# jeffsonyu/VTacO

Hardware: AMD Instinct MI355X
Metric: occupancy query-points/sec at 128^3 (decode stage, lattice -> logits on device) (higher is better)
Workload: dtype f16x3

## Files before the change

### include/vtaco_hip.h

```cpp
#ifndef VTACO_HIP_H
#define VTACO_HIP_H

#include <stddef.h>
#include <stdint.h>

#ifdef __cplusplus
extern "C" {
#endif

#define VT_ABI_VERSION 1

#define VT_ERR_INVALID      (-1)
#define VT_ERR_UNSUPPORTED  (-2)
#define VT_ERR_WORKSPACE    (-3)

#define VT_MAX_BLOCKS 8

int         vt_abi_version(void);
const char *vt_last_error(void);

typedef struct vt_decoder_params {
    int32_t hidden;
    int32_t c_dim;
    int32_t n_blocks;
// ... 38 lines not shown
                        int lattice_nx, float lattice_box, int64_t lattice_first,
                        const float *c_img, const unsigned char *finger_ids, const float *finger_feats, int F,
                        const float *blob_f16x3, double padding, float *out, float *out2, void *stream);

int vt_decoder_pack_f16f8(const vt_decoder_params *params_host, float *blob, size_t blob_bytes, void *stream);
int vt_decode_f16f8_covers(int R, int C, int lattice_nx, float lattice_box, int64_t lattice_first, int64_t N, double padding);
int vt_decode_fwd_f16f8(const float *grid_cl, int B, int R, int C, int64_t N,
                        int lattice_nx, float lattice_box, int64_t lattice_first,
                        const float *c_img, const unsigned char *finger_ids, const float *finger_feats, int F,
                        const float *blob_f16f8, double padding, float *out, void *stream);

int vt_decode_range_status(unsigned *host_status, int reset, void *stream);

int vt_decode_last_clock(unsigned long long *shader_cycles, unsigned long long *ref_ticks, int *ref_khz,
                         unsigned long long *wg_ticks, int max_wgs, int *n_wgs, void *stream);

#define VT_WIDE_LEAKY 1
#define VT_WIDE_NEAREST 2
size_t vt_decoder_wide_blob_bytes(int hidden, int c_dim, int n_blocks, int p_in);
int vt_decoder_pack_wide(const vt_decoder_params *params_host, float *blob, size_t blob_bytes, void *stream);
int vt_decode_fwd_wide(const float *grid_cl, int B, int R, int C, const float *pts, int64_t N,
                       int lattice_nx, float lattice_box, int64_t lattice_first,
                       const float *c_img, const float *blob_wide, int hidden, int n_blocks, int flags, double padding,
                       float *out, float *out2, void *stream);
size_t vt_decoder_wide_blob_f16x3_bytes(int hidden, int c_dim, int n_blocks, int p_in);
int vt_decoder_pack_wide_f16x3(const vt_decoder_params *params_host, float *blob, size_t blob_bytes, void *stream);
int vt_decode_fwd_wide_f16x3(const float *grid_cl, int B, int R, int C, const float *pts, int64_t N,
                             int lattice_nx, float lattice_box, int64_t lattice_first,
                             const float *c_img, const float *blob_wide_f16x3, int hidden, int n_blocks, int flags, double padding,
                             float *out, float *out2, void *stream);
// ... 488 lines not shown
```

### vtaco_amd/_lib.py

```python
from __future__ import annotations

import ctypes
import os

import torch

_HERE = os.path.dirname(os.path.abspath(__file__))
LIB_PATH = os.environ.get("VTACO_HIP_LIB") or os.path.join(_HERE, "libvtaco_hip.so")

VT_MAX_BLOCKS = 8
c_float_p = ctypes.POINTER(ctypes.c_float)


class VtError(RuntimeError):
    pass


class DecoderParams(ctypes.Structure):
    _fields_ = [
        ("hidden", ctypes.c_int32), ("c_dim", ctypes.c_int32),
        ("n_blocks", ctypes.c_int32), ("p_in", ctypes.c_int32),
        ("fc_p_w", ctypes.c_void_p), ("fc_p_b", ctypes.c_void_p),
        ("fc_c_w", ctypes.c_void_p * VT_MAX_BLOCKS), ("fc_c_b", ctypes.c_void_p * VT_MAX_BLOCKS),
        ("fc0_w", ctypes.c_void_p * VT_MAX_BLOCKS), ("fc0_b", ctypes.c_void_p * VT_MAX_BLOCKS),
# ... 117 lines not shown
    "vt_fusion_fwd_train": (_I, [_VP, _VP, _I, _I, ctypes.POINTER(FusionParams), _F, ctypes.c_ulonglong, _VP, _SZ, _VP, _SZ, _VP, _VP]),
    "vt_fusion_bwd": (_I, [_VP, _VP, _VP, _I, _I, ctypes.POINTER(FusionParams), _F, ctypes.c_ulonglong, _VP, _SZ, _VP, _SZ, _VP, _VP,
                           ctypes.POINTER(FusionGrads), _VP]),
    "vt_fusion_dropout_mask": (_I, [_F, ctypes.c_ulonglong, _I, _I, _I, _VP, _VP]),
    "vt_fusion_saved_bytes_wide": (_SZ, [_I, _I, _I]),
    "vt_fusion_bwd_workspace_bytes_wide": (_SZ, [_I, _I, _I]),
    "vt_fusion_dropout_mask_wide": (_I, [_F, ctypes.c_ulonglong, _I, _I, _I, _I, _VP, _VP]),
    "vt_decoder_blob_t_bytes": (_SZ, [_I, _I, _I]),
    "vt_decoder_pack_bf16x3": (_I, [ctypes.POINTER(DecoderParams), _VP, _SZ, _VP]),
    "vt_decode_fwd_bf16x3": (_I, [_VP, _I, _I, _I, _VP, _I64, _I, _F, _I64, _VP, _VP, _VP, _I, _VP, _D, _VP, _VP, _VP]),
    "vt_decoder_pack_f16x3": (_I, [ctypes.POINTER(DecoderParams), _VP, _SZ, _VP]),
    "vt_decode_fwd_f16x3": (_I, [_VP, _I, _I, _I, _VP, _I64, _I, _F, _I64, _VP, _VP, _VP, _I, _VP, _D, _VP, _VP, _VP]),
    "vt_decode_range_status": (_I, [ctypes.POINTER(ctypes.c_uint32), _I, _VP]),
    "vt_decode_last_clock": (_I, [ctypes.POINTER(ctypes.c_uint64), ctypes.POINTER(ctypes.c_uint64), ctypes.POINTER(ctypes.c_int),
                                  ctypes.POINTER(ctypes.c_uint64), _I, ctypes.POINTER(ctypes.c_int), _VP]),
    "vt_decoder_pack_f16f8": (_I, [ctypes.POINTER(DecoderParams), _VP, _SZ, _VP]),
    "vt_decoder_wide_blob_bytes": (_SZ, [_I, _I, _I, _I]),
    "vt_decoder_wide_blob_f16x3_bytes": (_SZ, [_I, _I, _I, _I]),
    "vt_decoder_pack_wide": (_I, [ctypes.POINTER(DecoderParams), _VP, _SZ, _VP]),
    "vt_decoder_pack_wide_f16x3": (_I, [ctypes.POINTER(DecoderParams), _VP, _SZ, _VP]),
    "vt_decode_fwd_wide": (_I, [_VP, _I, _I, _I, _VP, _I64, _I, _F, _I64, _VP, _VP, _I, _I, _I, _D, _VP, _VP, _VP]),
    "vt_decode_fwd_wide_f16x3": (_I, [_VP, _I, _I, _I, _VP, _I64, _I, _F, _I64, _VP, _VP, _I, _I, _I, _D, _VP, _VP, _VP]),
    "vt_decode_fwd_wide_ids": (_I, [_VP, _I, _I, _I, _VP, _I64, _I, _F, _I64, _VP, _VP, _I, _VP, _I, _I, _I, _D, _VP, _VP, _VP]),
    "vt_decode_wide_f16x3_workspace_bytes": (_SZ, [_I64, _I, _I, _I, _I]),
    "vt_decode_fwd_wide_f16x3_ws": (_I, [_VP, _I, _I, _I, _VP, _I64, _I, _F, _I64, _VP, _VP, _I, _I, _I, _D, _VP, _VP, _VP, _SZ, _VP]),
    "vt_decode_fwd_wide_f16x3_ids": (_I, [_VP, _I, _I, _I, _VP, _I64, _I, _F, _I64, _VP, _VP, _I, _VP, _I, _I, _I, _D, _VP, _VP, _VP]),
    "vt_decode_mlp_fwd_wide": (_I, [_VP, _I, _I, _VP, _I64, _I, _F, _I64, _VP, _I, _I, _I, _VP, _VP, _VP]),
    "vt_decode_mlp_fwd_wide_f16x3": (_I, [_VP, _I, _I, _VP, _I64, _I, _F, _I64, _VP, _I, _I, _I, _VP, _VP, _VP]),
    "vt_decode_wide_save_floats": (_SZ, [_I64, _I, _I, _I]),
    "vt_decode_wide_gws_floats": (_SZ, [_I64, _I, _I, _I]),
# ... 207 lines not shown
```

### vtaco_amd/csrc/decode.hip

```cpp
#include <hip/hip_runtime.h>
#include <atomic>
#include <mutex>
#include <type_traits>
#include <stdint.h>
#include <stdlib.h>

#include "decode_common.h"

namespace {

template <bool SAVE, int P>
__device__ __forceinline__ void mlp_and_heads(const DecodeArgs &a, const float *L, const f32x16 &c, float px, float py, float pz,
                                              uint32_t g, bool live, int lane, int h, bool with_img, unsigned &rmax) {
    const size_t slot = (size_t)a.total * 32;
    float *srow = SAVE ? a.save + (size_t)g * 32 : nullptr;
    if (SAVE && live) store_gather16(srow, c, h);

    f32x16 net = load_frag16(L + VT_OFF_BIAS + 0 * 32 + h * 16);
    {
        const float k0 = h ? py : px;
        const float k1 = h ? 0.0f : pz;
        net = mfma(L[VT_OFF_WP + lane], k0, net);
        net = mfma(L[VT_OFF_WP + 64 + lane], k1, net);
    }
// ... 368 lines not shown
    const int R = a.R;
    AxisEnt *tab = reinterpret_cast<AxisEnt *>(lds + VT_BLOB_FLOATS);
    for (int i = threadIdx.x; i < a.nx; i += ST2_THREADS) {
        float p, unused0, unused1;
        lattice_point(a, (uint32_t)i, 0u, 0u, p, unused0, unused1);
        const float f = grid_coord(p, a.divisor, R);
        const float f0 = floorf(f);
        AxisEnt e;
        e.i0 = (int)f0;
        e.w0 = (f0 + 1.0f) - f;
        e.i1 = min(e.i0 + 1, R - 1);
        e.w1 = (e.i0 + 1 <= R - 1) ? f - f0 : 0.0f;
        tab[i] = e;
    }
    unsigned *claim_ctr = reinterpret_cast<unsigned *>(reinterpret_cast<char *>(lds + VT_BLOB_FLOATS + 4 * a.nx) + (ST2_THREADS / 64) * ST2_WAVE_BYTES);
    if (threadIdx.x == 0) *claim_ctr = 0u;
    __syncthreads();

    const int lane = threadIdx.x & 63;
    const int pl = lane & 31;
    const int h = lane >> 5;
    const int wave = __builtin_amdgcn_readfirstlane(threadIdx.x >> 6);
    constexpr int WPB = ST2_THREADS / 64;
    const uint32_t ntiles = a.total >> 6;
    const uint32_t nx = (uint32_t)a.nx;
    const uint32_t tpb = a.N >> 6, q4 = nx >> 2, q8 = nx >> 3;
    const uint32_t plane0 = a.lattice_first / (nx * nx);
    char *stage = reinterpret_cast<char *>(lds + VT_BLOB_FLOATS + 4 * a.nx) + wave * ST2_WAVE_BYTES;

    uint32_t src_off[ST2_PIECES], dst_off[ST2_PIECES];
#pragma unroll
// ... 208 lines not shown
                netB = netB + bb;
            }
        }
        {
            const f32x16 wo = load_frag16(L + VT_OFF_OUT + h * 16);
            float accA = 0.0f, accB = 0.0f;
#pragma unroll
            for (int s = 0; s < 16; ++s) { accA = fmaf(relu1(netA[s]), wo[s], accA); accB = fmaf(relu1(netB[s]), wo[s], accB); }
            accA += __shfl_xor(accA, 32);
            accB += __shfl_xor(accB, 32);
            const float ob = L[VT_OFF_OUT + 64];
            if (h == 0) { a.out[gA] = accA + ob; a.out[gB] = accB + ob; }
        }
    }
    if constexpr (P == 2) range_report(rmax, a.status);
    clock_end(a.clk, stamp, reinterpret_cast<unsigned long long *>(claim_ctr + 4));
}

}
#ifdef VT_DECODE_F16_TU
#include "decode_st3.h"
#endif
namespace {

#ifndef VT_DECODE_F16_TU
__global__ void __launch_bounds__(256) sample_grid_kernel(DecodeArgs a, float *feat, int C) {
    const int lane = threadIdx.x & 63, pl = lane & 31, h = lane >> 5;
    const uint32_t ntiles = (a.total + 31u) >> 5;
    const int R = a.R;
    for (uint32_t tile = blockIdx.x * 4 + (threadIdx.x >> 6); tile < ntiles; tile += gridDim.x * 4) {
        uint32_t g = tile * 32u + pl;
// ... 196 lines not shown
        if (c0 + c < C && v0 + v < V) t[v][c] = s[(v0 + v) * C + c0 + c];
    }
    __syncthreads();
    for (int i = threadIdx.x; i < 32 * 64; i += 256) {
        const int c = i >> 6, v = i & 63;
        if (c0 + c < C && v0 + v < V) d[(int64_t)c * V + v0 + v] = t[v][c];
    }
}

#endif

}

#ifndef VT_DECODE_F16_TU
constexpr int VT_MAX_DEVICES = 64;
constexpr size_t VT_STATUS_BYTES = 8 + (4 + 2 * VT_CLK_MAX_WGS) * 8;
static std::mutex g_status_mutex;
static std::atomic<unsigned *> g_decode_status[VT_MAX_DEVICES];
unsigned *vt_decode_status_dev() {
    int dev = -1;
    if (hipGetDevice(&dev) != hipSuccess || dev < 0 || dev >= VT_MAX_DEVICES) return nullptr;
    unsigned *p = g_decode_status[dev].load(std::memory_order_acquire);
    if (p) return p;
    std::lock_guard<std::mutex> lock(g_status_mutex);
    p = g_decode_status[dev].load(std::memory_order_relaxed);
    if (!p) {
        if (hipMalloc(&p, VT_STATUS_BYTES) != hipSuccess) return nullptr;
        if (hipMemset(p, 0, VT_STATUS_BYTES) != hipSuccess) { (void)hipFree(p); return nullptr; }
        g_decode_status[dev].store(p, std::memory_order_release);
    }
    return p;
// ... 82 lines not shown
    if (e == hipSuccess) e = hipStreamSynchronize((hipStream_t)stream);
    int dev = 0, khz = 0;
    if (e == hipSuccess) e = hipGetDevice(&dev);
    if (e == hipSuccess) e = hipDeviceGetAttribute(&khz, hipDeviceAttributeWallClockRate, dev);
    if (e != hipSuccess) return vt_check(e, "vt_decode_last_clock");
    *shader_cycles = h[0]; *ref_ticks = h[1]; *ref_khz = khz;
    if (max_wgs > 0) {
        int n = (int)(h[2] < (unsigned long long)VT_CLK_MAX_WGS ? h[2] : VT_CLK_MAX_WGS);
        if (n > max_wgs) n = max_wgs;
        for (int i = 0; i < 2 * n; ++i) wg_ticks[i] = h[4 + i];
        *n_wgs = n;
    }
    return 0;
}

int vt_grid_to_channels_last(const float *src, float *dst, int B, int C, int D, int H, int W, void *stream) {
    if (!src || !dst || B <= 0 || C <= 0 || D <= 0 || H <= 0 || W <= 0) return vt_fail(VT_ERR_INVALID, "vt_grid_to_channels_last: bad argument");
    const int64_t V = (int64_t)D * H * W;
    dim3 grid((unsigned)((V + 63) / 64), (unsigned)((C + 31) / 32), (unsigned)B);
    hipLaunchKernelGGL(grid_to_cl_kernel, grid, dim3(256), 0, (hipStream_t)stream, src, dst, C, V);
    return vt_check(hipGetLastError(), "vt_grid_to_channels_last");
}

int vt_grid_from_channels_last(const float *src, float *dst, int B, int C, int D, int H, int W, void *stream) {
    if (!src || !dst || B <= 0 || C <= 0 || D <= 0 || H <= 0 || W <= 0) return vt_fail(VT_ERR_INVALID, "vt_grid_from_channels_last: bad argument");
    const int64_t V = (int64_t)D * H * W;
    dim3 grid((unsigned)((V + 63) / 64), (unsigned)((C + 31) / 32), (unsigned)B);
    hipLaunchKernelGGL(grid_from_cl_kernel, grid, dim3(256), 0, (hipStream_t)stream, src, dst, C, V);
    return vt_check(hipGetLastError(), "vt_grid_from_channels_last");
}
// ... 2 lines not shown
#endif

#ifdef VT_DECODE_F16_TU
static bool st3_covers(int nx, int R, double s_vox) {
    const size_t lds = ((size_t)VT_BLOB_FLOATS + 5u * (size_t)nx) * sizeof(float) + (size_t)(ST3_THREADS / 64) * ST2_WAVE_BYTES + VT_TAIL_LDS_BYTES;
    return (nx & 7) == 0 && R >= 6 && s_vox > 0.0 && s_vox < 0.55 && lds <= 160u * 1024u;
}
static int st3_launch(const DecodeArgs &a_in, int variant, void *stream) {
    DecodeArgs a = a_in;
    a.clk = status_clk(a.status);
    const size_t lds = ((size_t)VT_BLOB_FLOATS + 5u * (size_t)a.nx) * sizeof(float) + (size_t)(ST3_THREADS / 64) * ST2_WAVE_BYTES + VT_TAIL_LDS_BYTES;
    const int64_t nt = (int64_t)a.total / 64;
    int64_t blocks = (nt + ST3_THREADS / 64 - 1) / (ST3_THREADS / 64);
    if (blocks > vt_num_cus()) blocks = vt_num_cus();
    if (blocks > 8) blocks &= ~7ll;
    bool attr = false;
    if (!attr) {
        hipError_t e = vt_max_dyn_lds(reinterpret_cast<const void *>(&decode_fwd_staged3_kernel<0>), 160 * 1024);
        if (e == hipSuccess) e = vt_max_dyn_lds(reinterpret_cast<const void *>(&decode_fwd_staged3_kernel<1>), 160 * 1024);
        if (e == hipSuccess) e = vt_max_dyn_lds(reinterpret_cast<const void *>(&decode_fwd_staged3_kernel<2>), 160 * 1024);
        if (e == hipSuccess) e = vt_max_dyn_lds(reinterpret_cast<const void *>(&decode_fwd_staged3_kernel<3>), 160 * 1024);
        if (e != hipSuccess) return vt_check(e, "vt_decode_fwd: hipFuncSetAttribute (staged3)");
        attr = true;
    }
    if (variant == 0) hipLaunchKernelGGL(decode_fwd_staged3_kernel<0>, dim3((unsigned)blocks), dim3(ST3_THREADS), lds, (hipStream_t)stream, a);
    else if (variant == 1) hipLaunchKernelGGL(decode_fwd_staged3_kernel<1>, dim3((unsigned)blocks), dim3(ST3_THREADS), lds, (hipStream_t)stream, a);
    else if (variant == 2) hipLaunchKernelGGL(decode_fwd_staged3_kernel<2>, dim3((unsigned)blocks), dim3(ST3_THREADS), lds, (hipStream_t)stream, a);
    else hipLaunchKernelGGL(decode_fwd_staged3_kernel<3>, dim3((unsigned)blocks), dim3(ST3_THREADS), lds, (hipStream_t)stream, a);
    return vt_check(hipGetLastError(), "vt_decode_fwd");
}
static double lattice_step_voxels(int R, int nx, float box, double padding) {
    return (double)(R - 1) * (double)box / ((double)(nx - 1) * (double)(float)(1.0 + padding + 10e-4));
}
int vt_st3_sample_lattice(const float *grid_cl, int B, int R, int C, int64_t N, int nx, float box, int64_t first, double padding,
                          float *feat, void *stream, int *covered) {
    *covered = 0;
    if (C != 32 || nx < 8 || N <= 0 || (int64_t)B * N >= (int64_t)1 << 31) return 0;
    const int64_t pair = 2ll * nx * nx;
// ... 243 lines not shown
```

### vtaco_amd/csrc/decode_common.h

```cpp
#pragma once
#include <hip/hip_runtime.h>
#include <stdint.h>

#include "vt_common.h"

namespace {

typedef float f32x16 __attribute__((ext_vector_type(16)));
typedef float f32x4 __attribute__((ext_vector_type(4)));

__device__ __forceinline__ f32x16 mfma(float a, float b, f32x16 c) {
    return __builtin_amdgcn_mfma_f32_32x32x2f32(a, b, c, 0, 0, 0);
}

__device__ __forceinline__ float relu1(float x) {
    return __builtin_amdgcn_fmed3f(x, 0.0f, __builtin_inff());
}

__device__ __forceinline__ void pin16(f32x16 &v) {
    asm volatile("" : "+v"(v));
}

template <bool RELU>
__device__ __forceinline__ f32x16 dense32(f32x16 acc, const float *wl, const f32x16 &x, int lane) {
// ... 99 lines not shown
}

constexpr int VT_CLK_MAX_WGS = 512;
constexpr unsigned VT_TAIL_LDS_BYTES = 256;
struct ClockStamp {
    unsigned long long t0, r0;
};
__device__ __forceinline__ ClockStamp clock_begin(const unsigned long long *clk) {
    ClockStamp c{0ull, 0ull};
    if (clk != nullptr) {
        c.r0 = __builtin_amdgcn_s_memrealtime();
        if (blockIdx.x == 0) c.t0 = __builtin_readcyclecounter();
    }
    return c;
}
__device__ __forceinline__ void clock_end(unsigned long long *clk, const ClockStamp &c, unsigned long long *wave_ends) {
    if (clk != nullptr) {
        const unsigned long long r1 = __builtin_amdgcn_s_memrealtime();
        const unsigned long long dt = blockIdx.x == 0 ? __builtin_readcyclecounter() - c.t0 : 0ull;
        const int nwaves = (int)(blockDim.x >> 6);
        if ((threadIdx.x & 63) == 0) wave_ends[threadIdx.x >> 6] = r1;
        __syncthreads();
        if (threadIdx.x == 0) {
            unsigned long long last = r1;
            for (int w = 1; w < nwaves; ++w) last = wave_ends[w] > last ? wave_ends[w] : last;
            if (blockIdx.x == 0) { clk[0] = dt; clk[1] = r1 - c.r0; clk[2] = gridDim.x; }
            if (blockIdx.x < VT_CLK_MAX_WGS) { clk[4 + 2 * blockIdx.x] = c.r0; clk[5 + 2 * blockIdx.x] = last; }
        }
    }
}

template <int P>
__device__ __forceinline__ f32x16 dense32s(f32x16 acc, const float *wl, const SplitP<P> &x, int lane) {
    const mx8<P> *w = reinterpret_cast<const mx8<P> *>(wl);
#pragma unroll
    for (int s = 0; s < 2; ++s) {
        const mx8<P> wh = w[s * 64 + lane], wo = w[(2 + s) * 64 + lane];
        acc = mfma_s(wo, x.hi[s], acc);
        acc = mfma_s(wh, x.lo[s], acc);
        acc = mfma_s(wh, x.hi[s], acc);
    }
    return acc;
// ... 136 lines not shown
```

### vtaco_amd/csrc/decode_st3.h

```cpp
#pragma once

namespace {

typedef unsigned u32x8 __attribute__((ext_vector_type(8)));
typedef int i32x8 __attribute__((ext_vector_type(8)));
typedef short i16x2 __attribute__((ext_vector_type(2)));

constexpr int ST3_F8_SX = VT_F8_SX;
constexpr int ST3_F8_SW = VT_F8_SW;

template <int V> struct SpT {
    u32x4 hi[2], lo[2];
};
template <> struct SpT<2> {
    u32x4 hi[2];
    u32x8 q;
};

__device__ __forceinline__ f32x16 mfma_h(const u32x4 &a, const u32x4 &b, f32x16 c) {
    return __builtin_amdgcn_mfma_f32_32x32x16_f16(__builtin_bit_cast(f16x8, a), __builtin_bit_cast(f16x8, b), c, 0, 0, 0);
}
__device__ __forceinline__ f32x16 mfma_q(const u32x8 &a, const u32x8 &b, f32x16 c) {
    return __builtin_amdgcn_mfma_scale_f32_32x32x64_f8f6f4(__builtin_bit_cast(i32x8, a), __builtin_bit_cast(i32x8, b), c, 0, 0,
                                                           0, 127 - 11 - ST3_F8_SW, 0, 127 + ST3_F8_SX);
// ... 96 lines not shown
static_assert(ST3_CHUNKS - 64 * ST3_PIECES == 8, "the last LDS-DMA piece is eight lanes");

#define ST3_GAP() __builtin_amdgcn_sched_barrier(0)
#define ST3_M(acc, w, x) do { acc = mfma_h(w, x, acc); ST3_GAP(); } while (0)
#define ST3_Q(acc, w, x) do { acc = mfma_q(w, x, acc); ST3_GAP(); } while (0)
#define ST3_RUN_BLOCKS() do { _Pragma("unroll 1") for (int i = 0; i < 4; ++i) block(i, std::true_type{}); block(4, std::false_type{}); } while (0)
#define ST3_S(dst, src, k) split_step<V, true, k>(dst, src, m1, rmax)
#define ST3_C(dst, src, k) split_step<V, false, k>(dst, src, m1, rmax)

template <int V>
__global__ void __launch_bounds__(ST3_THREADS)
decode_fwd_staged3_kernel(DecodeArgs a) {
    extern __shared__ __attribute__((aligned(16))) float lds[];
    const ClockStamp stamp = clock_begin(a.clk);
    if constexpr (V == 2) __builtin_amdgcn_s_setreg((1 - 1) << 11 | 23 << 6 | 1, 1);
    if constexpr (V != 3) {
        const f32x4 *src = reinterpret_cast<const f32x4 *>(a.blob);
        f32x4 *dst = reinterpret_cast<f32x4 *>(lds);
        for (int i = threadIdx.x; i < VT_BLOB_FLOATS / 4; i += ST3_THREADS) dst[i] = src[i];
    }
    const int R = a.R;
    AxisEnt *tab = reinterpret_cast<AxisEnt *>(lds + VT_BLOB_FLOATS);
    unsigned *ptab = reinterpret_cast<unsigned *>(tab + a.nx);
    for (int i = threadIdx.x; i < a.nx; i += ST3_THREADS) {
        float p, unused0, unused1;
        lattice_point(a, (uint32_t)i, 0u, 0u, p, unused0, unused1);
        const float f = grid_coord(p, a.divisor, R);
        const float f0 = floorf(f);
        AxisEnt e;
        e.i0 = (int)f0;
        e.w0 = (f0 + 1.0f) - f;
        e.i1 = min(e.i0 + 1, R - 1);
        e.w1 = (e.i0 + 1 <= R - 1) ? f - f0 : 0.0f;
        tab[i] = e;
        const _Float16 ph = (_Float16)p;
        const _Float16 pm = (_Float16)(p - (float)ph);
        ptab[i] = (unsigned)__builtin_bit_cast(unsigned short, ph) | ((unsigned)__builtin_bit_cast(unsigned short, pm) << 16);
    }
    if (threadIdx.x == 0)
        *reinterpret_cast<unsigned *>(reinterpret_cast<char *>(lds + VT_BLOB_FLOATS + 5 * a.nx) + (ST3_THREADS / 64) * ST2_WAVE_BYTES) = 0u;
    __syncthreads();

    const int lane = threadIdx.x & 63;
    const int pl = lane & 31;
    const int h = lane >> 5;
    const int wave = __builtin_amdgcn_readfirstlane(threadIdx.x >> 6);
    constexpr int WPB = ST3_THREADS / 64;
    const uint32_t ntiles = a.total >> 6;
    const uint32_t nx = (uint32_t)a.nx;
    const uint32_t tpb = a.N >> 6, q4 = nx >> 2, q8 = nx >> 3;
    const uint32_t plane0 = a.lattice_first / (nx * nx);
    char *stage = reinterpret_cast<char *>(lds + VT_BLOB_FLOATS + 5 * a.nx) + wave * ST2_WAVE_BYTES;
    unsigned *claim_ctr = reinterpret_cast<unsigned *>(reinterpret_cast<char *>(lds + VT_BLOB_FLOATS + 5 * a.nx) + WPB * ST2_WAVE_BYTES);
    const unsigned stage_lds = (unsigned)__builtin_amdgcn_readfirstlane((int)(unsigned)reinterpret_cast<size_t>(stage));
    const unsigned stage_lds_last = (unsigned)__builtin_amdgcn_readfirstlane((int)(stage_lds + 1024u * ST3_PIECES));

    uint32_t src_off[ST3_PIECES + 1];
#pragma unroll
    for (int k = 0; k <= ST3_PIECES; ++k) {
        const int m = min(64 * k + lane, ST3_CHUNKS - 1), row = m / 9, c = m - 9 * row;
        const int dx = row % 3, t = row / 3, dy = t & 3, dz = t >> 2;
        src_off[k] = (uint32_t)((dz * R + dy) * R + dx) * 128u + (uint32_t)((c == 8) ? 0 : c) * 16u;
    }

    uint32_t t_begin = 0, t_end = ntiles, w_idx = blockIdx.x * WPB + wave, w_cnt = gridDim.x * WPB;
    if ((gridDim.x & 7u) == 0 && ntiles >= 8u * WPB) {
        const uint32_t chunk = (ntiles + 7u) >> 3, xcd = blockIdx.x & 7u;
        t_begin = min(xcd * chunk, ntiles);
        t_end = min(t_begin + chunk, ntiles);
        w_idx = (blockIdx.x >> 3) * WPB + wave;
        w_cnt = (gridDim.x >> 3) * WPB;
    }
    auto brick_of = [&](uint32_t tile, uint32_t &b, uint32_t &X0, uint32_t &Y0, uint32_t &Z0) {
        b = tile / tpb;
        const uint32_t t = tile - b * tpb;
        const uint32_t pp = t / (q4 * q8), rem = t - pp * q4 * q8;
        const uint32_t by = rem / q8, bz = rem - by * q8;
        X0 = 2u * pp; Y0 = 4u * by; Z0 = 8u * bz;
    };
    int ox = 0, oy = 0, oz = 0;
    auto fetch = [&](uint32_t tile, int &fx, int &fy, int &fz) {
        uint32_t b, X0, Y0, Z0;
        brick_of(tile, b, X0, Y0, Z0);
        fx = min(__builtin_amdgcn_readfirstlane(tab[plane0 + X0].i0), R - 3);
        fy = min(__builtin_amdgcn_readfirstlane(tab[Y0].i0), R - 4);
        fz = min(__builtin_amdgcn_readfirstlane(tab[Z0].i0), R - 6);
        const uint64_t bp = reinterpret_cast<uint64_t>(a.grid + ((((size_t)b * R + fz) * R + fy) * R + fx) * 32);
        const char *base = reinterpret_cast<const char *>(
            ((uint64_t)(uint32_t)__builtin_amdgcn_readfirstlane((int)(bp >> 32)) << 32) |
            (uint64_t)(uint32_t)__builtin_amdgcn_readfirstlane((int)(uint32_t)bp));
        unsigned keep;
        asm volatile(
            "s_mov_b32 %[keep], m0\n\t"
            "s_nop 4\n\t"
            "s_mov_b32 m0, %[dst]\n\ts_nop 0\n\tglobal_load_lds_dwordx4 %[o0], %[base]\n\t"
            "s_add_u32 m0, m0, 0x400\n\ts_nop 0\n\tglobal_load_lds_dwordx4 %[o1], %[base]\n\t"
            "s_add_u32 m0, m0, 0x400\n\ts_nop 0\n\tglobal_load_lds_dwordx4 %[o2], %[base]\n\t"
            "s_add_u32 m0, m0, 0x400\n\ts_nop 0\n\tglobal_load_lds_dwordx4 %[o3], %[base]\n\t"
            "s_add_u32 m0, m0, 0x400\n\ts_nop 0\n\tglobal_load_lds_dwordx4 %[o4], %[base]\n\t"
            "s_add_u32 m0, m0, 0x400\n\ts_nop 0\n\tglobal_load_lds_dwordx4 %[o5], %[base]\n\t"
            "s_add_u32 m0, m0, 0x400\n\ts_nop 0\n\tglobal_load_lds_dwordx4 %[o6], %[base]\n\t"
// ... 5 lines not shown
            : [dst] "s"(stage_lds), [base] "s"(base), [o0] "v"(src_off[0]), [o1] "v"(src_off[1]), [o2] "v"(src_off[2]),
              [o3] "v"(src_off[3]), [o4] "v"(src_off[4]), [o5] "v"(src_off[5]), [o6] "v"(src_off[6]), [o7] "v"(src_off[7]),
              [o8] "v"(src_off[8]), [o9] "v"(src_off[9])
            : "memory", "scc");
        if (lane < ST3_CHUNKS - 64 * ST3_PIECES) {
            asm volatile(
                "s_mov_b32 %[keep], m0\n\t"
                "s_nop 4\n\t"
                "s_mov_b32 m0, %[dst]\n\ts_nop 0\n\tglobal_load_lds_dwordx4 %[o], %[base]\n\t"
                "s_mov_b32 m0, %[keep]"
                : [keep] "=&s"(keep)
                : [dst] "s"(stage_lds_last), [base] "s"(base), [o] "v"(src_off[ST3_PIECES])
                : "memory");
        }
    };

    u32x4 ones;
    {
        f16x8 o;
#pragma unroll
        for (int e = 0; e < 8; ++e) o[e] = (_Float16)((h == 0 && e < 3) ? 1.0f : 0.0f);
        ones = __builtin_bit_cast(u32x4, o);
    }
    const float m1 = opaque_minus_one();
    unsigned rmax = 0;
    [[maybe_unused]] float lmax = 0.0f;

    const uint32_t wg_first = t_begin + w_idx - (uint32_t)wave;
    unsigned fixed_next = (unsigned)wave;
    auto claim = [&]() -> uint32_t {
        unsigned i = 0;
        if (!a.claim) { i = fixed_next; fixed_next += (unsigned)WPB; }
        else {
            if (lane == 0) i = __hip_atomic_fetch_add(claim_ctr, 1u, __ATOMIC_RELAXED, __HIP_MEMORY_SCOPE_WORKGROUP);
            i = (unsigned)__builtin_amdgcn_readfirstlane((int)i);
        }
        const uint32_t t = wg_first + (i % (unsigned)WPB) + (i / (unsigned)WPB) * w_cnt;
        return i < 0x10000u ? t : t_end;
    };
    uint32_t tile = claim();
    if (tile < t_end) fetch(tile, ox, oy, oz);
    uint32_t next_tile = t_end;
    for (; tile < t_end; tile = next_tile) {
        unsigned lds_off = 0;
        asm volatile("" : "+v"(lds_off));
        const float *L = lds + lds_off;

        uint32_t b, X0, Y0, Z0;
        brick_of(tile, b, X0, Y0, Z0);
        const uint32_t ixl = X0 + (uint32_t)(pl >> 4), iy = Y0 + (uint32_t)((pl >> 2) & 3), izA = Z0 + (uint32_t)(pl & 3), izB = izA + 4u;
        const uint32_t gA = b * a.N + (ixl * nx + iy) * nx + izA, gB = gA + 4u;
        const AxisEnt ex = tab[plane0 + ixl], ey = tab[iy], ezA = tab[izA], ezB = tab[izB];
        const unsigned img_lds = stage_lds + 64u * (unsigned)h;
        const unsigned cx0 = (unsigned)(ex.i0 - ox) * ST_ROW_BYTES, cx1 = (unsigned)(ex.i1 - ox) * ST_ROW_BYTES;
        const unsigned cy0 = (unsigned)(ey.i0 - oy) * (3u * ST_ROW_BYTES) + img_lds, cy1 = (unsigned)(ey.i1 - oy) * (3u * ST_ROW_BYTES) + img_lds;
        const unsigned c00 = cy0 + cx0, c01 = cy0 + cx1, c10 = cy1 + cx0, c11 = cy1 + cx1;
        const float w00 = ex.w0 * ey.w0, w01 = ex.w1 * ey.w0, w10 = ex.w0 * ey.w1, w11 = ex.w1 * ey.w1;
// ... 82 lines not shown
                    const u32x4 ih0 = frag(VT_OFF_WPI), ih1 = frag(VT_OFF_WPI + 256);
                    const u32x8 iq = frag8(VT_OFF_WPI + 512);
                    netA = mfma_h(ih0, iA.hi[0], netA); netB = mfma_h(ih0, iB.hi[0], netB);
                    netA = mfma_h(ih1, iA.hi[1], netA); netB = mfma_h(ih1, iB.hi[1], netB);
                    netA = mfma_q(iq, iA.q, netA); netB = mfma_q(iq, iB.q, netB);
                } else {
                    dense32s2<2>(netA, netB, L + VT_OFF_WPI, split16<false, 2>(ciA), split16<false, 2>(ciB), lane);
                }
            }
        }

        u32x4 w0h0, w0h1, w1h0, w1h1, ch0, ch1, bf;
        [[maybe_unused]] u32x4 w0o0, w0o1, w1o0, w1o1, co0, co1;
        [[maybe_unused]] u32x8 w0q, w1q, cq;
        f32x16 hidA, hidB;
        if constexpr (V == 2) {
#include "decode_st3_f16f8.inc"
            ST3_RUN_BLOCKS();
        } else {
#include "decode_st3_f16x3.inc"
            ST3_RUN_BLOCKS();
        }
        }
    }
    range_report(rmax, a.status, V == 2);
    if constexpr (V == 2) {
        if (a.status != nullptr && lmax > VT_F16F8_LOGIT_LIMIT) atomicOr(a.status, VT_RANGE_LOGIT);
    }
    clock_end(a.clk, stamp, reinterpret_cast<unsigned long long *>(claim_ctr + 4));
}

#undef ST3_GAP
#undef ST3_M
#undef ST3_S
#undef ST3_C

}
```

### vtaco_amd/csrc/decode_st3_f16f8.inc

```
        {
            const u32x4 wp = frag(VT_OFF_PFRAG);
            u32x4 f0h0 = frag(VT_OFF_WL), f0h1 = frag(VT_OFF_WL + 256); u32x8 f0q = frag8(VT_OFF_WL + 512);
            ST3_M(netA, wp, pA);
            ST3_C(csA, cA, 0);
            ST3_C(csA, cA, 1);
            ST3_C(csA, cA, 2);
            ST3_GAP();
            ST3_M(netA, f0h0, csA.hi[0]);
            ST3_C(csA, cA, 3);
            ST3_C(csA, cA, 4);
            ST3_C(csA, cA, 5);
            ST3_C(csA, cA, 6);
            ST3_GAP();
            ST3_M(netA, f0h1, csA.hi[1]);
            ST3_C(csA, cA, 7);
            ST3_C(csB, cB, 0);
            ST3_C(csB, cB, 1);
            ST3_GAP();
            ST3_Q(netA, f0q, csA.q);
            ST3_C(csB, cB, 2);
            ST3_C(csB, cB, 3);
            ST3_C(csB, cB, 4);
            ST3_GAP();
            ST3_M(netB, wp, pB);
// ... 174 lines not shown
                ST3_GAP();
            } else {
                const f32x16 wo = load_frag16(L + VT_OFF_OUT + h * 16);
                const float ob = L[VT_OFF_OUT + 64];
                float accA = 0.0f, accB = 0.0f;
                ST3_M(netB, w1h0, sB.hi[0]);
                ST3_GAP();
                ST3_M(netB, w1h1, sB.hi[1]);
#pragma unroll
                for (int s = 0; s < 8; ++s) accA = fmaf(relu1(netA[s]), wo[s], accA);
                ST3_GAP();
                ST3_Q(netB, w1q, sB.q);
#pragma unroll
                for (int s = 8; s < 16; ++s) accA = fmaf(relu1(netA[s]), wo[s], accA);
                accA += __shfl_xor(accA, 32);
                if (h == 0) a.out[gA] = accA + ob;
                lmax = fmaxf(lmax, fabsf(accA + ob));
                ST3_GAP();
#pragma unroll
                for (int s = 0; s < 16; ++s) accB = fmaf(relu1(netB[s]), wo[s], accB);
                accB += __shfl_xor(accB, 32);
                if (h == 0) a.out[gB] = accB + ob;
                lmax = fmaxf(lmax, fabsf(accB + ob));
            }
        };
```

### vtaco_amd/csrc/decode_st3_f16x3.inc

```
        {
            const u32x4 wp = frag(VT_OFF_PFRAG);
            u32x4 f0h0 = frag(VT_OFF_WL), f0h1 = frag(VT_OFF_WL + 256), f0o0 = frag(VT_OFF_WL + 512), f0o1 = frag(VT_OFF_WL + 768);
            ST3_M(netA, wp, pA);
            ST3_C(csA, cA, 0);
            ST3_C(csA, cA, 1);
            ST3_C(csA, cA, 2);
            ST3_C(csA, cA, 3);
            ST3_C(csA, cA, 4);
            ST3_GAP();
            ST3_M(netA, f0o0, csA.hi[0]);
            ST3_C(csA, cA, 5);
            ST3_GAP();
            ST3_M(netA, f0h0, csA.lo[0]);
            ST3_C(csA, cA, 6);
            ST3_GAP();
            ST3_M(netA, f0h0, csA.hi[0]);
            ST3_C(csA, cA, 7);
            ST3_GAP();
            ST3_M(netA, f0o1, csA.hi[1]);
            ST3_C(csB, cB, 0);
            ST3_C(csB, cB, 1);
            ST3_GAP();
            ST3_M(netA, f0h1, csA.lo[1]);
            ST3_C(csB, cB, 2);
// ... 257 lines not shown
#pragma unroll
                for (int s = 4; s < 7; ++s) accA = fmaf(relu1(netA[s]), wo[s], accA);
                ST3_GAP();
                ST3_M(netB, w1o1, sB.hi[1]);
#pragma unroll
                for (int s = 7; s < 10; ++s) accA = fmaf(relu1(netA[s]), wo[s], accA);
                ST3_GAP();
                ST3_M(netB, w1h1, sB.lo[1]);
#pragma unroll
                for (int s = 10; s < 13; ++s) accA = fmaf(relu1(netA[s]), wo[s], accA);
                ST3_GAP();
                ST3_M(netB, w1h1, sB.hi[1]);
#pragma unroll
                for (int s = 13; s < 16; ++s) accA = fmaf(relu1(netA[s]), wo[s], accA);
                accA += __shfl_xor(accA, 32);
                if (h == 0) a.out[gA] = accA + ob;
                ST3_GAP();
#pragma unroll
                for (int s = 0; s < 16; ++s) accB = fmaf(relu1(netB[s]), wo[s], accB);
                accB += __shfl_xor(accB, 32);
                if (h == 0) a.out[gB] = accB + ob;
            }
        };
```

### vtaco_amd/csrc/gen_st3.py

```python
#!/usr/bin/env python3
import os

HERE = os.path.dirname(os.path.abspath(__file__))


def M(acc, w, x):
    return f"ST3_M({acc}, {w}, {x});"


def Q(acc, w, x):
    return f"ST3_Q({acc}, {w}, {x});"


class Mode:
    def __init__(self, name):
        self.name = name
        self.f8 = name == "f16f8"

    def layer(self, acc, w, x):
        if self.f8:
            return [M(acc, f"{w}h0", f"{x}.hi[0]"), M(acc, f"{w}h1", f"{x}.hi[1]"), Q(acc, f"{w}q", f"{x}.q")]
        return [M(acc, f"{w}o0", f"{x}.hi[0]"), M(acc, f"{w}h0", f"{x}.lo[0]"), M(acc, f"{w}h0", f"{x}.hi[0]"),
                M(acc, f"{w}o1", f"{x}.hi[1]"), M(acc, f"{w}h1", f"{x}.lo[1]"), M(acc, f"{w}h1", f"{x}.hi[1]")]

# ... 131 lines not shown
                float accA = 0.0f, accB = 0.0f;
""")
    pm = md.layer("netB", "w1", "sB")
    n = len(pm)
    gaps = list(range(1, n))
    per = [16 // len(gaps) + (1 if g < 16 % len(gaps) else 0) for g in range(len(gaps))]
    lo = 0
    for j, m in enumerate(pm):
        o.append(I3 + m + "\n")
        if j in gaps:
            cnt = per[gaps.index(j)]
            o.append("#pragma unroll\n")
            o.append(I3 + f"for (int s = {lo}; s < {lo + cnt}; ++s) accA = fmaf(relu1(netA[s]), wo[s], accA);\n")
            lo += cnt
        if j == n - 1:
            o.append(I3 + "accA += __shfl_xor(accA, 32);\n" + I3 + "if (h == 0) a.out[gA] = accA + ob;\n")
            if md.f8:
                o.append(I3 + "lmax = fmaxf(lmax, fabsf(accA + ob));                       // the logit-scale guard of the fp8 form\n")
        o.append(I3 + "ST3_GAP();\n")
    o.append("""#pragma unroll
                for (int s = 0; s < 16; ++s) accB = fmaf(relu1(netB[s]), wo[s], accB);
                accB += __shfl_xor(accB, 32);
                if (h == 0) a.out[gB] = accB + ob;
""" + ("                lmax = fmaxf(lmax, fabsf(accB + ob));\n" if md.f8 else "") + """            }
        };
""")
    with open(os.path.join(HERE, f"decode_st3_{mode}.inc"), "w") as f:
        f.write("".join(o))


if __name__ == "__main__":
    generate("f16x3")
    generate("f16f8")
    print("wrote decode_st3_f16x3.inc, decode_st3_f16f8.inc")
```

### vtaco_amd/ops.py

```python
from __future__ import annotations

import ctypes
import os
from collections import namedtuple

import torch

from . import _lib
from ._lib import VtError, check, dev_ptr, stream_ptr


_graph_keep = None


class graph_keepalive:

    def __enter__(self):
        global _graph_keep
        self._prev, _graph_keep = _graph_keep, []
        return _graph_keep

    def __exit__(self, *exc):
        global _graph_keep
        _graph_keep = self._prev
# ... 112 lines not shown
                                           stream_ptr()), "vt_decode_last_clock")
    if ref.value == 0 or khz.value <= 0:
        return None
    tick_us = 1e3 / khz.value
    us = ref.value * tick_us
    res = {"shader_mhz": cyc.value / us, "wg0_us": us, "shader_cycles": int(cyc.value), "ref_khz": int(khz.value)}
    if workgroups and n.value > 0:
        st = [(buf[2 * i], buf[2 * i + 1]) for i in range(n.value)]
        t0 = min(a for a, _ in st)
        dur = sorted((b - a) * tick_us for a, b in st)
        res.update({"workgroups": n.value, "span_us": (max(b for _, b in st) - t0) * tick_us,
                    "start_spread_us": (max(a for a, _ in st) - t0) * tick_us,
                    "wg_us_min": dur[0], "wg_us_median": dur[len(dur) // 2], "wg_us_max": dur[-1],
                    "wg_ticks": [[int(a - t0), int(b - t0)] for a, b in st]})
    return res


def is_channels_last_grid(grid):
    B, C, D, H, W = grid.shape
    return grid.stride() == (D * H * W * C, 1, H * W * C, W * C, C)


def grid_to_channels_last(grid):
    if is_channels_last_grid(grid):
        return grid
    g = grid.detach()
    if not g.is_contiguous():
        g = g.contiguous()
    B, C, D, H, W = g.shape
    out = torch.empty((B, D, H, W, C), dtype=torch.float32, device=g.device)
# ... 2149 lines not shown
```

Baseline: 12.74 billion.

## Overlap first tile fetch with blob staging and use nontemporal logit stores

The staged3 decode kernel now issues each wave's first grid-tile fetch before staging the weight blob, computing that tile's origin directly instead of reading it from the axis table. The blob copy into LDS now uses asynchronous global_load_lds pieces, so the prologue latency overlaps with the first tile load. Logit output stores become nontemporal, and the attribute setup is cached per device. The change also adds per-workgroup phase-timing instrumentation (MFMA start/end, last claim) and replaces the end-of-kernel barrier in clock_end with LDS atomics; these add some overhead only when clocking is enabled.

```diff
diff --git a/include/vtaco_hip.h b/include/vtaco_hip.h
--- a/include/vtaco_hip.h
+++ b/include/vtaco_hip.h
@@ -76,6 +76,7 @@
 
 int vt_decode_last_clock(unsigned long long *shader_cycles, unsigned long long *ref_ticks, int *ref_khz,
                          unsigned long long *wg_ticks, int max_wgs, int *n_wgs, void *stream);
+int vt_decode_last_phases(unsigned long long *wg_phase_ticks, int max_wgs, int *n_wgs, void *stream);
 
 #define VT_WIDE_LEAKY 1
 #define VT_WIDE_NEAREST 2
diff --git a/vtaco_amd/_lib.py b/vtaco_amd/_lib.py
--- a/vtaco_amd/_lib.py
+++ b/vtaco_amd/_lib.py
@@ -155,6 +155,7 @@
     "vt_decode_range_status": (_I, [ctypes.POINTER(ctypes.c_uint32), _I, _VP]),
     "vt_decode_last_clock": (_I, [ctypes.POINTER(ctypes.c_uint64), ctypes.POINTER(ctypes.c_uint64), ctypes.POINTER(ctypes.c_int),
                                   ctypes.POINTER(ctypes.c_uint64), _I, ctypes.POINTER(ctypes.c_int), _VP]),
+    "vt_decode_last_phases": (_I, [ctypes.POINTER(ctypes.c_uint64), _I, ctypes.POINTER(ctypes.c_int), _VP]),
     "vt_decoder_pack_f16f8": (_I, [ctypes.POINTER(DecoderParams), _VP, _SZ, _VP]),
     "vt_decoder_wide_blob_bytes": (_SZ, [_I, _I, _I, _I]),
     "vt_decoder_wide_blob_f16x3_bytes": (_SZ, [_I, _I, _I, _I]),
diff --git a/vtaco_amd/csrc/decode.hip b/vtaco_amd/csrc/decode.hip
--- a/vtaco_amd/csrc/decode.hip
+++ b/vtaco_amd/csrc/decode.hip
@@ -406,7 +406,7 @@
         tab[i] = e;
     }
     unsigned *claim_ctr = reinterpret_cast<unsigned *>(reinterpret_cast<char *>(lds + VT_BLOB_FLOATS + 4 * a.nx) + (ST2_THREADS / 64) * ST2_WAVE_BYTES);
-    if (threadIdx.x == 0) *claim_ctr = 0u;
+    if (threadIdx.x == 0) clock_tail_init(reinterpret_cast<ClockTail *>(claim_ctr), 0u);
     __syncthreads();
 
     const int lane = threadIdx.x & 63;
@@ -645,7 +645,7 @@
         }
     }
     if constexpr (P == 2) range_report(rmax, a.status);
-    clock_end(a.clk, stamp, reinterpret_cast<unsigned long long *>(claim_ctr + 4));
+    clock_end(a.clk, stamp, reinterpret_cast<ClockTail *>(claim_ctr));
 }
 
 }
@@ -872,7 +872,7 @@
 
 #ifndef VT_DECODE_F16_TU
 constexpr int VT_MAX_DEVICES = 64;
-constexpr size_t VT_STATUS_BYTES = 8 + (4 + 2 * VT_CLK_MAX_WGS) * 8;
+constexpr size_t VT_STATUS_BYTES = 8 + (4 + 5 * VT_CLK_MAX_WGS) * 8;
 static std::mutex g_status_mutex;
 static std::atomic<unsigned *> g_decode_status[VT_MAX_DEVICES];
 unsigned *vt_decode_status_dev() {
@@ -985,6 +985,21 @@
     return 0;
 }
 
+int vt_decode_last_phases(unsigned long long *wg_phase_ticks, int max_wgs, int *n_wgs, void *stream) {
+    if (max_wgs <= 0 || !wg_phase_ticks || !n_wgs) return vt_fail(VT_ERR_INVALID, "vt_decode_last_phases: bad workgroup buffer");
+    unsigned *d = vt_decode_status_dev();
+    if (!d) return vt_fail(VT_ERR_INVALID, "vt_decode_last_phases: no device memory for the status block");
+    static thread_local unsigned long long h[4 + 5 * VT_CLK_MAX_WGS];
+    hipError_t e = hipMemcpyAsync(h, status_clk(d), sizeof(h), hipMemcpyDeviceToHost, (hipStream_t)stream);
+    if (e == hipSuccess) e = hipStreamSynchronize((hipStream_t)stream);
+    if (e != hipSuccess) return vt_check(e, "vt_decode_last_phases");
+    int n = (int)(h[2] < (unsigned long long)VT_CLK_MAX_WGS ? h[2] : VT_CLK_MAX_WGS);
+    if (n > max_wgs) n = max_wgs;
+    for (int i = 0; i < 3 * n; ++i) wg_phase_ticks[i] = h[4 + 2 * VT_CLK_MAX_WGS + i];
+    *n_wgs = n;
+    return 0;
+}
+
 int vt_grid_to_channels_last(const float *src, float *dst, int B, int C, int D, int H, int W, void *stream) {
     if (!src || !dst || B <= 0 || C <= 0 || D <= 0 || H <= 0 || W <= 0) return vt_fail(VT_ERR_INVALID, "vt_grid_to_channels_last: bad argument");
     const int64_t V = (int64_t)D * H * W;
@@ -1017,14 +1032,17 @@
     int64_t blocks = (nt + ST3_THREADS / 64 - 1) / (ST3_THREADS / 64);
     if (blocks > vt_num_cus()) blocks = vt_num_cus();
     if (blocks > 8) blocks &= ~7ll;
-    bool attr = false;
-    if (!attr) {
+    constexpr int MAX_DEVICES = 64;
+    static std::atomic<bool> attr[MAX_DEVICES];
+    int dev = -1;
+    if (hipGetDevice(&dev) != hipSuccess || dev < 0 || dev >= MAX_DEVICES) return vt_fail(VT_ERR_INVALID, "vt_decode_fwd: no current device");
+    if (!attr[dev].load(std::memory_order_acquire)) {
         hipError_t e = vt_max_dyn_lds(reinterpret_cast<const void *>(&decode_fwd_staged3_kernel<0>), 160 * 1024);
         if (e == hipSuccess) e = vt_max_dyn_lds(reinterpret_cast<const void *>(&decode_fwd_staged3_kernel<1>), 160 * 1024);
         if (e == hipSuccess) e = vt_max_dyn_lds(reinterpret_cast<const void *>(&decode_fwd_staged3_kernel<2>), 160 * 1024);
         if (e == hipSuccess) e = vt_max_dyn_lds(reinterpret_cast<const void *>(&decode_fwd_staged3_kernel<3>), 160 * 1024);
         if (e != hipSuccess) return vt_check(e, "vt_decode_fwd: hipFuncSetAttribute (staged3)");
-        attr = true;
+        attr[dev].store(true, std::memory_order_release);
     }
     if (variant == 0) hipLaunchKernelGGL(decode_fwd_staged3_kernel<0>, dim3((unsigned)blocks), dim3(ST3_THREADS), lds, (hipStream_t)stream, a);
     else if (variant == 1) hipLaunchKernelGGL(decode_fwd_staged3_kernel<1>, dim3((unsigned)blocks), dim3(ST3_THREADS), lds, (hipStream_t)stream, a);
diff --git a/vtaco_amd/csrc/decode_common.h b/vtaco_amd/csrc/decode_common.h
--- a/vtaco_amd/csrc/decode_common.h
+++ b/vtaco_amd/csrc/decode_common.h
@@ -137,18 +137,47 @@
     }
     return c;
 }
-__device__ __forceinline__ void clock_end(unsigned long long *clk, const ClockStamp &c, unsigned long long *wave_ends) {
+struct ClockTail {
+    unsigned claim;
+    unsigned arrived;
+    unsigned long long end;
+    unsigned long long mfma_first, mfma_last;
+    unsigned long long last_claim;
+};
+static_assert(sizeof(ClockTail) <= VT_TAIL_LDS_BYTES, "the tail words fit behind the images");
+__device__ __forceinline__ void clock_tail_init(ClockTail *t, unsigned first_claim) {
+    t->claim = first_claim; t->arrived = 0u; t->end = 0ull; t->mfma_first = ~0ull; t->mfma_last = 0ull; t->last_claim = 0ull;
+}
+__device__ __forceinline__ void clock_mark_mfma(const unsigned long long *clk, ClockTail *t) {
+    if (clk != nullptr) {
+        const unsigned long long r = __builtin_amdgcn_s_memrealtime();
+        if ((threadIdx.x & 63) == 0) {
+            __hip_atomic_fetch_min(&t->mfma_first, r, __ATOMIC_RELAXED, __HIP_MEMORY_SCOPE_WORKGROUP);
+            __hip_atomic_fetch_max(&t->mfma_last, r, __ATOMIC_RELAXED, __HIP_MEMORY_SCOPE_WORKGROUP);
+        }
+    }
+}
+__device__ __forceinline__ void clock_mark_claim(const unsigned long long *clk, ClockTail *t) {
+    if (clk != nullptr) {
+        const unsigned long long r = __builtin_amdgcn_s_memrealtime();
+        if ((threadIdx.x & 63) == 0) __hip_atomic_fetch_max(&t->last_claim, r, __ATOMIC_RELAXED, __HIP_MEMORY_SCOPE_WORKGROUP);
+    }
+}
+__device__ __forceinline__ void clock_end(unsigned long long *clk, const ClockStamp &c, ClockTail *t) {
     if (clk != nullptr) {
         const unsigned long long r1 = __builtin_amdgcn_s_memrealtime();
-        const unsigned long long dt = blockIdx.x == 0 ? __builtin_readcyclecounter() - c.t0 : 0ull;
-        const int nwaves = (int)(blockDim.x >> 6);
-        if ((threadIdx.x & 63) == 0) wave_ends[threadIdx.x >> 6] = r1;
-        __syncthreads();
-        if (threadIdx.x == 0) {
-            unsigned long long last = r1;
-            for (int w = 1; w < nwaves; ++w) last = wave_ends[w] > last ? wave_ends[w] : last;
-            if (blockIdx.x == 0) { clk[0] = dt; clk[1] = r1 - c.r0; clk[2] = gridDim.x; }
-            if (blockIdx.x < VT_CLK_MAX_WGS) { clk[4 + 2 * blockIdx.x] = c.r0; clk[5 + 2 * blockIdx.x] = last; }
+        if ((threadIdx.x & 63) == 0) {
+            if (threadIdx.x == 0 && blockIdx.x == 0) {
+                clk[0] = __builtin_readcyclecounter() - c.t0; clk[1] = r1 - c.r0; clk[2] = gridDim.x;
+            }
+            __hip_atomic_fetch_max(&t->end, r1, __ATOMIC_RELAXED, __HIP_MEMORY_SCOPE_WORKGROUP);
+            const unsigned before = __hip_atomic_fetch_add(&t->arrived, 1u, __ATOMIC_ACQ_REL, __HIP_MEMORY_SCOPE_WORKGROUP);
+            if (before + 1u == (blockDim.x >> 6) && blockIdx.x < VT_CLK_MAX_WGS) {
+                clk[4 + 2 * blockIdx.x] = c.r0;
+                clk[5 + 2 * blockIdx.x] = __hip_atomic_load(&t->end, __ATOMIC_RELAXED, __HIP_MEMORY_SCOPE_WORKGROUP);
+                unsigned long long *ph = clk + 4 + 2 * VT_CLK_MAX_WGS + 3 * blockIdx.x;
+                ph[0] = t->mfma_first; ph[1] = t->mfma_last; ph[2] = t->last_claim;
+            }
         }
     }
 }
diff --git a/vtaco_amd/csrc/decode_st3.h b/vtaco_amd/csrc/decode_st3.h
--- a/vtaco_amd/csrc/decode_st3.h
+++ b/vtaco_amd/csrc/decode_st3.h
@@ -134,33 +134,9 @@
     extern __shared__ __attribute__((aligned(16))) float lds[];
     const ClockStamp stamp = clock_begin(a.clk);
     if constexpr (V == 2) __builtin_amdgcn_s_setreg((1 - 1) << 11 | 23 << 6 | 1, 1);
-    if constexpr (V != 3) {
-        const f32x4 *src = reinterpret_cast<const f32x4 *>(a.blob);
-        f32x4 *dst = reinterpret_cast<f32x4 *>(lds);
-        for (int i = threadIdx.x; i < VT_BLOB_FLOATS / 4; i += ST3_THREADS) dst[i] = src[i];
-    }
     const int R = a.R;
     AxisEnt *tab = reinterpret_cast<AxisEnt *>(lds + VT_BLOB_FLOATS);
     unsigned *ptab = reinterpret_cast<unsigned *>(tab + a.nx);
-    for (int i = threadIdx.x; i < a.nx; i += ST3_THREADS) {
-        float p, unused0, unused1;
-        lattice_point(a, (uint32_t)i, 0u, 0u, p, unused0, unused1);
-        const float f = grid_coord(p, a.divisor, R);
-        const float f0 = floorf(f);
-        AxisEnt e;
-        e.i0 = (int)f0;
-        e.w0 = (f0 + 1.0f) - f;
-        e.i1 = min(e.i0 + 1, R - 1);
-        e.w1 = (e.i0 + 1 <= R - 1) ? f - f0 : 0.0f;
-        tab[i] = e;
-        const _Float16 ph = (_Float16)p;
-        const _Float16 pm = (_Float16)(p - (float)ph);
-        ptab[i] = (unsigned)__builtin_bit_cast(unsigned short, ph) | ((unsigned)__builtin_bit_cast(unsigned short, pm) << 16);
-    }
-    if (threadIdx.x == 0)
-        *reinterpret_cast<unsigned *>(reinterpret_cast<char *>(lds + VT_BLOB_FLOATS + 5 * a.nx) + (ST3_THREADS / 64) * ST2_WAVE_BYTES) = 0u;
-    __syncthreads();
-
     const int lane = threadIdx.x & 63;
     const int pl = lane & 31;
     const int h = lane >> 5;
@@ -171,7 +147,8 @@
     const uint32_t tpb = a.N >> 6, q4 = nx >> 2, q8 = nx >> 3;
     const uint32_t plane0 = a.lattice_first / (nx * nx);
     char *stage = reinterpret_cast<char *>(lds + VT_BLOB_FLOATS + 5 * a.nx) + wave * ST2_WAVE_BYTES;
-    unsigned *claim_ctr = reinterpret_cast<unsigned *>(reinterpret_cast<char *>(lds + VT_BLOB_FLOATS + 5 * a.nx) + WPB * ST2_WAVE_BYTES);
+    ClockTail *tail = reinterpret_cast<ClockTail *>(reinterpret_cast<char *>(lds + VT_BLOB_FLOATS + 5 * a.nx) + WPB * ST2_WAVE_BYTES);
+    unsigned *claim_ctr = &tail->claim;
     const unsigned stage_lds = (unsigned)__builtin_amdgcn_readfirstlane((int)(unsigned)reinterpret_cast<size_t>(stage));
     const unsigned stage_lds_last = (unsigned)__builtin_amdgcn_readfirstlane((int)(stage_lds + 1024u * ST3_PIECES));
 
@@ -199,12 +176,7 @@
         X0 = 2u * pp; Y0 = 4u * by; Z0 = 8u * bz;
     };
     int ox = 0, oy = 0, oz = 0;
-    auto fetch = [&](uint32_t tile, int &fx, int &fy, int &fz) {
-        uint32_t b, X0, Y0, Z0;
-        brick_of(tile, b, X0, Y0, Z0);
-        fx = min(__builtin_amdgcn_readfirstlane(tab[plane0 + X0].i0), R - 3);
-        fy = min(__builtin_amdgcn_readfirstlane(tab[Y0].i0), R - 4);
-        fz = min(__builtin_amdgcn_readfirstlane(tab[Z0].i0), R - 6);
+    auto fetch_at = [&](uint32_t b, int fx, int fy, int fz) {
         const uint64_t bp = reinterpret_cast<uint64_t>(a.grid + ((((size_t)b * R + fz) * R + fy) * R + fx) * 32);
         const char *base = reinterpret_cast<const char *>(
             ((uint64_t)(uint32_t)__builtin_amdgcn_readfirstlane((int)(bp >> 32)) << 32) |
@@ -240,6 +212,69 @@
                 : "memory");
         }
     };
+    auto fetch = [&](uint32_t tile, int &fx, int &fy, int &fz) {
+        uint32_t b, X0, Y0, Z0;
+        brick_of(tile, b, X0, Y0, Z0);
+        fx = min(__builtin_amdgcn_readfirstlane(tab[plane0 + X0].i0), R - 3);
+        fy = min(__builtin_amdgcn_readfirstlane(tab[Y0].i0), R - 4);
+        fz = min(__builtin_amdgcn_readfirstlane(tab[Z0].i0), R - 6);
+        fetch_at(b, fx, fy, fz);
+    };
+
+    const uint32_t wg_first = t_begin + w_idx - (uint32_t)wave;
+    uint32_t tile = min(wg_first + (uint32_t)wave, t_end);
+    if (tile < t_end) {
+        auto axis_i0 = [&](uint32_t i) {
+            float p, unused0, unused1;
+            lattice_point(a, i, 0u, 0u, p, unused0, unused1);
+            return __builtin_amdgcn_readfirstlane((int)floorf(grid_coord(p, a.divisor, R)));
+        };
+        uint32_t b, X0, Y0, Z0;
+        brick_of(tile, b, X0, Y0, Z0);
+        ox = min(axis_i0(plane0 + X0), R - 3);
+        oy = min(axis_i0(Y0), R - 4);
+        oz = min(axis_i0(Z0), R - 6);
+        fetch_at(b, ox, oy, oz);
+        if (tile + w_cnt >= t_end) clock_mark_claim(a.clk, tail);
+    }
+    if constexpr (V != 3) {
+        constexpr unsigned BLOB_BYTES = (unsigned)VT_BLOB_FLOATS * 4u, FULL = BLOB_BYTES / 1024u, REST_LANES = (BLOB_BYTES % 1024u) / 16u;
+        static_assert(BLOB_BYTES % 16u == 0, "the blob is whole 16-byte chunks");
+        const unsigned lds0 = (unsigned)__builtin_amdgcn_readfirstlane((int)(unsigned)reinterpret_cast<size_t>(lds));
+        const char *blob = reinterpret_cast<const char *>(a.blob);
+        const uint32_t voff = (uint32_t)lane * 16u;
+        auto piece = [&](unsigned k) {
+            unsigned keep;
+            asm volatile(
+                "s_mov_b32 %[keep], m0\n\t"
+                "s_nop 4\n\t"
+                "s_mov_b32 m0, %[dst]\n\ts_nop 0\n\tglobal_load_lds_dwordx4 %[o], %[base]\n\t"
+                "s_mov_b32 m0, %[keep]"
+                : [keep] "=&s"(keep)
+                : [dst] "s"(lds0 + 1024u * k), [base] "s"(blob + 1024u * k), [o] "v"(voff)
+                : "memory");
+        };
+        for (unsigned k = (unsigned)wave; k < FULL; k += (unsigned)WPB) piece(k);
+        if (REST_LANES != 0u && wave == (int)(FULL % (unsigned)WPB) && lane < (int)REST_LANES) piece(FULL);
+    }
+    for (int i = threadIdx.x; i < a.nx; i += ST3_THREADS) {
+        float p, unused0, unused1;
+        lattice_point(a, (uint32_t)i, 0u, 0u, p, unused0, unused1);
+        const float f = grid_coord(p, a.divisor, R);
+        const float f0 = floorf(f);
+        AxisEnt e;
+        e.i0 = (int)f0;
+        e.w0 = (f0 + 1.0f) - f;
+        e.i1 = min(e.i0 + 1, R - 1);
+        e.w1 = (e.i0 + 1 <= R - 1) ? f - f0 : 0.0f;
+        tab[i] = e;
+        const _Float16 ph = (_Float16)p;
+        const _Float16 pm = (_Float16)(p - (float)ph);
+        ptab[i] = (unsigned)__builtin_bit_cast(unsigned short, ph) | ((unsigned)__builtin_bit_cast(unsigned short, pm) << 16);
+    }
+    if (threadIdx.x == 0) clock_tail_init(tail, (unsigned)WPB);
+    asm volatile("s_waitcnt vmcnt(0)" ::: "memory");
+    __syncthreads();
 
     u32x4 ones;
     {
@@ -252,8 +287,7 @@
     unsigned rmax = 0;
     [[maybe_unused]] float lmax = 0.0f;
 
-    const uint32_t wg_first = t_begin + w_idx - (uint32_t)wave;
-    unsigned fixed_next = (unsigned)wave;
+    unsigned fixed_next = (unsigned)(wave + WPB);
     auto claim = [&]() -> uint32_t {
         unsigned i = 0;
         if (!a.claim) { i = fixed_next; fixed_next += (unsigned)WPB; }
@@ -262,11 +296,11 @@
             i = (unsigned)__builtin_amdgcn_readfirstlane((int)i);
         }
         const uint32_t t = wg_first + (i % (unsigned)WPB) + (i / (unsigned)WPB) * w_cnt;
+        if (i < 0x10000u && t < t_end && t + w_cnt >= t_end) clock_mark_claim(a.clk, tail);
         return i < 0x10000u ? t : t_end;
     };
-    uint32_t tile = claim();
-    if (tile < t_end) fetch(tile, ox, oy, oz);
     uint32_t next_tile = t_end;
+    [[maybe_unused]] bool mfma_marked = false;
     for (; tile < t_end; tile = next_tile) {
         unsigned lds_off = 0;
         asm volatile("" : "+v"(lds_off));
@@ -379,6 +413,7 @@
         [[maybe_unused]] u32x4 w0o0, w0o1, w1o0, w1o1, co0, co1;
         [[maybe_unused]] u32x8 w0q, w1q, cq;
         f32x16 hidA, hidB;
+        if (!mfma_marked) { clock_mark_mfma(a.clk, tail); mfma_marked = true; }
         if constexpr (V == 2) {
 #include "decode_st3_f16f8.inc"
             ST3_RUN_BLOCKS();
@@ -392,7 +427,7 @@
     if constexpr (V == 2) {
         if (a.status != nullptr && lmax > VT_F16F8_LOGIT_LIMIT) atomicOr(a.status, VT_RANGE_LOGIT);
     }
-    clock_end(a.clk, stamp, reinterpret_cast<unsigned long long *>(claim_ctr + 4));
+    clock_end(a.clk, stamp, tail);
 }
 
 #undef ST3_GAP
diff --git a/vtaco_amd/csrc/decode_st3_f16f8.inc b/vtaco_amd/csrc/decode_st3_f16f8.inc
--- a/vtaco_amd/csrc/decode_st3_f16f8.inc
+++ b/vtaco_amd/csrc/decode_st3_f16f8.inc
@@ -212,13 +212,13 @@
 #pragma unroll
                 for (int s = 8; s < 16; ++s) accA = fmaf(relu1(netA[s]), wo[s], accA);
                 accA += __shfl_xor(accA, 32);
-                if (h == 0) a.out[gA] = accA + ob;
+                if (h == 0) __builtin_nontemporal_store(accA + ob, a.out + gA);
                 lmax = fmaxf(lmax, fabsf(accA + ob));
                 ST3_GAP();
 #pragma unroll
                 for (int s = 0; s < 16; ++s) accB = fmaf(relu1(netB[s]), wo[s], accB);
                 accB += __shfl_xor(accB, 32);
-                if (h == 0) a.out[gB] = accB + ob;
+                if (h == 0) __builtin_nontemporal_store(accB + ob, a.out + gB);
                 lmax = fmaxf(lmax, fabsf(accB + ob));
             }
         };
diff --git a/vtaco_amd/csrc/decode_st3_f16x3.inc b/vtaco_amd/csrc/decode_st3_f16x3.inc
--- a/vtaco_amd/csrc/decode_st3_f16x3.inc
+++ b/vtaco_amd/csrc/decode_st3_f16x3.inc
@@ -295,11 +295,11 @@
 #pragma unroll
                 for (int s = 13; s < 16; ++s) accA = fmaf(relu1(netA[s]), wo[s], accA);
                 accA += __shfl_xor(accA, 32);
-                if (h == 0) a.out[gA] = accA + ob;
+                if (h == 0) __builtin_nontemporal_store(accA + ob, a.out + gA);
                 ST3_GAP();
 #pragma unroll
                 for (int s = 0; s < 16; ++s) accB = fmaf(relu1(netB[s]), wo[s], accB);
                 accB += __shfl_xor(accB, 32);
-                if (h == 0) a.out[gB] = accB + ob;
+                if (h == 0) __builtin_nontemporal_store(accB + ob, a.out + gB);
             }
         };
diff --git a/vtaco_amd/csrc/gen_st3.py b/vtaco_amd/csrc/gen_st3.py
--- a/vtaco_amd/csrc/gen_st3.py
+++ b/vtaco_amd/csrc/gen_st3.py
@@ -169,14 +169,14 @@
             o.append(I3 + f"for (int s = {lo}; s < {lo + cnt}; ++s) accA = fmaf(relu1(netA[s]), wo[s], accA);\n")
             lo += cnt
         if j == n - 1:
-            o.append(I3 + "accA += __shfl_xor(accA, 32);\n" + I3 + "if (h == 0) a.out[gA] = accA + ob;\n")
+            o.append(I3 + "accA += __shfl_xor(accA, 32);\n" + I3 + "if (h == 0) __builtin_nontemporal_store(accA + ob, a.out + gA);\n")
             if md.f8:
                 o.append(I3 + "lmax = fmaxf(lmax, fabsf(accA + ob));                       // the logit-scale guard of the fp8 form\n")
         o.append(I3 + "ST3_GAP();\n")
     o.append("""#pragma unroll
                 for (int s = 0; s < 16; ++s) accB = fmaf(relu1(netB[s]), wo[s], accB);
                 accB += __shfl_xor(accB, 32);
-                if (h == 0) a.out[gB] = accB + ob;
+                if (h == 0) __builtin_nontemporal_store(accB + ob, a.out + gB);
 """ + ("                lmax = fmaxf(lmax, fabsf(accB + ob));\n" if md.f8 else "") + """            }
         };
 """)
diff --git a/vtaco_amd/ops.py b/vtaco_amd/ops.py
--- a/vtaco_amd/ops.py
+++ b/vtaco_amd/ops.py
@@ -150,6 +150,23 @@
                     "wg_us_min": dur[0], "wg_us_median": dur[len(dur) // 2], "wg_us_max": dur[-1],
                     "wg_ticks": [[int(a - t0), int(b - t0)] for a, b in st]})
     return res
+
+
+def decode_last_phases():
+    n, m = ctypes.c_int(0), ctypes.c_int(0)
+    cyc, ref, khz = ctypes.c_uint64(0), ctypes.c_uint64(0), ctypes.c_int(0)
+    wg, ph = (ctypes.c_uint64 * 1024)(), (ctypes.c_uint64 * 1536)()
+    lib = _lib.load()
+    check(lib.vt_decode_last_clock(ctypes.byref(cyc), ctypes.byref(ref), ctypes.byref(khz), wg, 512, ctypes.byref(n), stream_ptr()),
+          "vt_decode_last_clock")
+    check(lib.vt_decode_last_phases(ph, 512, ctypes.byref(m), stream_ptr()), "vt_decode_last_phases")
+    if n.value == 0 or m.value != n.value or khz.value <= 0:
+        return None
+    rows = [[wg[2 * i], ph[3 * i], ph[3 * i + 1], ph[3 * i + 2], wg[2 * i + 1]] for i in range(n.value)]
+    if any(r[1] == 2 ** 64 - 1 or r[2] == 0 or r[3] == 0 for r in rows):
+        return None
+    t0 = min(r[0] for r in rows)
+    return {"ref_khz": int(khz.value), "wg_phase_ticks": [[int(v - t0) for v in r] for r in rows]}
 
 
 def is_channels_last_grid(grid):
```

Result: no change. 12.80 billion, median of 6 (+0.5%).
